# Ensembl/WiggleTools

Measured on AMD Instinct MI355X. Metric: genomic bp/s (whole node) for 'mean' over N BigWig tracks, higher is better.
Workload: dtype f64

## Files before the change

wiggletools_amd/csrc/wt_engine.hip:

```cpp
#include <hip/hip_runtime.h>

#include <cstdio>
#include <thread>
#include <atomic>
#include <cstring>
#include <map>
#include <mutex>
#include <string>
#include <vector>

#include "wt_host.h"
#include "wt_trackset.h"
#include "wt_core.h"
#include "wt_plan.h"
#include "wt_kernels.h"
#include "wt_devscope.h"
#include "wt_pool.h"

#ifndef WT_INDEX_UNROLL
#define WT_INDEX_UNROLL 2
#endif
#define WT_INDEX_CHUNK (256 * 4 * WT_INDEX_UNROLL)
__global__ void __launch_bounds__(256) wt_index_kernel(const WtParams P, long long total, long long span) {
    const long long dev_total = P.seg_off[(long long) P.n_chrom * P.n_tracks];
    if (total > dev_total) total = dev_total;
    const long long begin0 = (long long) blockIdx.x * span;
    long long end0 = begin0 + span;
    if (end0 > total) end0 = total;
    if (begin0 >= end0) return;
    WtIndexCursor cur;
    wt_index_cursor_set(P, cur, wt_index_find_segment(P, begin0));
    struct __attribute__((packed, aligned(4))) V4 { int32_t x[4]; };
    V4 f[WT_INDEX_UNROLL], nf[WT_INDEX_UNROLL];
    int32_t pf[WT_INDEX_UNROLL], npf[WT_INDEX_UNROLL];
    const long long n_full = (end0 - begin0) / WT_INDEX_CHUNK;
    auto fetch = [&](long long base, V4 (&v)[WT_INDEX_UNROLL], int32_t (&p)[WT_INDEX_UNROLL]) {
#pragma unroll
        for (int u = 0; u < WT_INDEX_UNROLL; u++) {
            const long long g = base + 4ll * (threadIdx.x + 256 * u);
            v[u] = *(const V4 *) (P.finish + g);
            p[u] = P.finish[g > 0 ? g - 1 : 0];
        }
    };
    if (n_full > 0) {
        const long long last_full = begin0 + (n_full - 1) * WT_INDEX_CHUNK;
        fetch(begin0, f, pf);
        for (long long begin = begin0; begin <= last_full; begin += WT_INDEX_CHUNK) {
            const long long nb = begin + WT_INDEX_CHUNK;
            fetch(nb <= last_full ? nb : last_full, nf, npf);
#pragma unroll
            for (int u = 0; u < WT_INDEX_UNROLL; u++) {
                const long long g = begin + 4ll * (threadIdx.x + 256 * u);
                int32_t prev = pf[u];
#pragma unroll
                for (int q = 0; q < 4; q++) {
                    wt_index_apply(P, cur, g + q, f[u].x[q], prev);
                    prev = f[u].x[q];
                }
            }
#pragma unroll
            for (int u = 0; u < WT_INDEX_UNROLL; u++) { f[u] = nf[u]; pf[u] = npf[u]; }
        }
    }
    const long long begin = begin0 + n_full * WT_INDEX_CHUNK;
    if (begin < end0) {
#pragma unroll
        for (int u = 0; u < WT_INDEX_UNROLL; u++) {
            const long long g = begin + 4ll * (threadIdx.x + 256 * u);
            int32_t prev = (g < end0 && g > 0) ? P.finish[g - 1] : 0;
#pragma unroll
            for (int q = 0; q < 4; q++) {
                if (g + q < end0) {
                    const int32_t fq = P.finish[g + q];
                    wt_index_apply(P, cur, g + q, fq, prev);
                    prev = fq;
                }
            }
        }
    }
}

#define WT_ISEARCH_ROWS 64
#define WT_ISEARCH_TRACKS 16

__device__ __forceinline__ int wt_index_row_chrom(const WtParams &P, long long row) {
    int lo = 0;
    for (int hi = P.n_chrom; hi - lo > 1;) {
        const int mid = (lo + hi) >> 1;
        if (P.c_first_win[mid] + mid <= row) lo = mid; else hi = mid;
    }
    return lo;
}

struct WtIndexRow { int ch; long long b, s0, n; };
__device__ __forceinline__ WtIndexRow wt_index_row(const WtParams &P, long long row, int i) {
    WtIndexRow r;
    r.ch = P.n_chrom == 1 ? 0 : wt_index_row_chrom(P, row);
    const long long m = row - (P.c_first_win[r.ch] + r.ch);
    const long long seg = (long long) r.ch * P.n_tracks + i;
    r.s0 = P.seg_off[seg];
    r.n = P.seg_off[seg + 1] - r.s0;
    r.b = (long long) P.cbase[r.ch] + (m << P.logW);
    return r;
}

__global__ void __launch_bounds__(256) wt_index_coarse_kernel(const WtParams P, long long n_strips, uint32_t *coarse) {
    const long long t = (long long) blockIdx.x * 256 + threadIdx.x;
    const int N = P.n_tracks;
    if (t >= n_strips * N) return;
    const long long strip = t / N;
    const int i = (int) (t - strip * N);
    const WtIndexRow r = wt_index_row(P, strip * WT_ISEARCH_ROWS, i);
    const int32_t *fin = P.finish + r.s0;
    long long g = r.n >> 1;
    float density = 0.0f;
    if (r.n > 1) {
        const long long f0 = fin[0], f1 = fin[r.n - 1];
        if (f1 > f0) {
            density = (float) (r.n - 1) / (float) (f1 - f0);
            const float guess = fminf(fmaxf((float) (r.b - f0) * density, 0.0f), (float) (r.n - 1));
            g = (long long) guess;
            if (g > r.n - 1) g = r.n - 1;
        }
    }
    coarse[t] = (uint32_t) wt_interp_lower_bound(WtFinArray{fin}, 0, r.n, g, r.b, density);
}

__global__ void __launch_bounds__(WT_ISEARCH_ROWS * WT_ISEARCH_TRACKS) wt_index_search_kernel(const WtParams P, long long n_rows, long long n_strips,
                                                                                              const uint32_t *coarse) {
    __shared__ uint32_t out[WT_ISEARCH_ROWS][WT_ISEARCH_TRACKS + 1];
    const int tid = threadIdx.x, lane = tid & 63;
    const int wave = __builtin_amdgcn_readfirstlane(tid >> 6);
    const int N = P.n_tracks;
    const long long strip = blockIdx.x;
    const long long r0 = strip * WT_ISEARCH_ROWS;
    const int i = (int) blockIdx.y * WT_ISEARCH_TRACKS + wave;
    if (i < N) {
        long long row = r0 + lane;
        if (row > n_rows - 1) row = n_rows - 1;
        const WtIndexRow r = wt_index_row(P, row, i);
        const int32_t *fin = P.finish + r.s0;
        const bool have_next = strip + 1 < n_strips;
        const long long cA = (long long) coarse[strip * N + i];
        const long long cB = have_next ? (long long) coarse[(strip + 1) * N + i] : 0;
        bool real_a = true, real_b = have_next;
        if (P.n_chrom != 1) {
            const int ch_first = __shfl(r.ch, 0);
            const int ch_next = have_next ? wt_index_row_chrom(P, r0 + WT_ISEARCH_ROWS) : -1;
            real_a = r.ch == ch_first; real_b = r.ch == ch_next;
        }
        const long long A = real_a ? cA : 0;
        const long long B = real_b ? cB : r.n;
        long long g = (real_a && real_b) ? A + (((B - A) * lane) >> 6) : (A + B) >> 1;
        if (g > B - 1) g = B - 1;
        const float density = (real_a && real_b) ? (float) (B - A) / (float) ((long long) WT_ISEARCH_ROWS << P.logW) : 0.0f;
        out[lane][wave] = (uint32_t) wt_interp_lower_bound(WtFinArray{fin}, A, B, g, r.b, density);
    }
    __syncthreads();
    const int orow = tid / WT_ISEARCH_TRACKS, ocol = tid % WT_ISEARCH_TRACKS;
    const long long row = r0 + orow;
    const int track = (int) blockIdx.y * WT_ISEARCH_TRACKS + ocol;
    if (row < n_rows && track < N) P.widx[(size_t) row * N + track] = out[orow][ocol];
}

__global__ void __launch_bounds__(256) wt_index_compare_kernel(const uint32_t *a, const uint32_t *b, long long n, unsigned long long *diff) {
    const long long t = (long long) blockIdx.x * 256 + threadIdx.x;
    if (t < n && a[t] != b[t]) atomicAdd(diff, 1ull);
}

__global__ void __launch_bounds__(256) wt_extents_kernel(const int64_t *seg_off, const int32_t *start,
                                                          const int32_t *finish, long long n_seg,
                                                          int32_t *first_start, int32_t *last_finish) {
    const long long s = (long long) blockIdx.x * blockDim.x + threadIdx.x;
    if (s >= n_seg) return;
    const long long lo = seg_off[s], hi = seg_off[s + 1];
    first_start[s] = hi > lo ? start[lo] : 0;
    last_finish[s] = hi > lo ? finish[hi - 1] : 0;
}

__global__ void __launch_bounds__(256) wt_win_chrom_kernel(const int64_t *c_first_win, int n_chrom, long long n_windows, int32_t *win_chrom) {
    const long long k = (long long) blockIdx.x * 256 + threadIdx.x;
    if (k >= n_windows) return;
    int lo = 0;
    for (int hi = n_chrom; hi - lo > 1;) {
        const int mid = (lo + hi) >> 1;
        if (c_first_win[mid] <= k) lo = mid; else hi = mid;
    }
    win_chrom[k] = lo;
}

__global__ void __launch_bounds__(256) wt_clear_kernel(unsigned long long *counters, int n_counters, int64_t *chrom_run_off, int n_cro,
                                                        unsigned long long *status, long long n_status) {
    const long long t = (long long) blockIdx.x * 256 + threadIdx.x, stride = (long long) gridDim.x * 256;
    for (long long q = t; q < n_status; q += stride) status[q] = 0ull;
    for (long long q = t; q < n_counters; q += stride) counters[q] = 0ull;
    for (long long q = t; q < n_cro; q += stride) chrom_run_off[q] = 0;
}

__global__ void __launch_bounds__(256) wt_validate_kernel(const int32_t *start, const int32_t *finish, const int64_t *seg_off,
                                                           long long n_seg, long long total, unsigned long long *out) {
    const long long g = (long long) blockIdx.x * blockDim.x + threadIdx.x;
    if (g >= total) return;
    bool bad = finish[g] <= start[g];
    if (!bad && g > 0 && start[g] < finish[g - 1]) {
        long long lo = 0, hi = n_seg;
        while (hi - lo > 1) {
            const long long mid = (lo + hi) >> 1;
            if (seg_off[mid] <= g) lo = mid; else hi = mid;
        }
        bad = seg_off[lo] != g;
    }
    if (bad) {
        atomicAdd(&out[0], 1ull);
        atomicMin(&out[1], (unsigned long long) g);
    }
}

static thread_local std::string g_last_error;

int wt_fail(int code, const std::string &msg) {
    g_last_error = msg;
    return code;
}

template <class T>
static hipError_t wt_grow(T **p, int64_t *cap, int64_t need, bool *quiet) {
    if (*cap >= need && *p) return hipSuccess;
    int64_t c = *cap * 2;
    if (c < need) c = need;
    if (c < 1) c = 1;
    if (*p) {
        if (!*quiet) {
            const hipError_t eq = wt_pool_quiesce();
            if (eq != hipSuccess) return eq;
            *quiet = true;
        }
        (void) wt_dev_free(*p);
    }
    *p = nullptr; *cap = 0;
    const hipError_t e = wt_dev_alloc(p, sizeof(T) * (size_t) c);
    if (e == hipSuccess) *cap = c;
    return e;
}

static void wt_free_windows(WtWindows &w) {
    (void) wt_dev_free(w.d_tabs);
    (void) wt_dev_free(w.d_widx); (void) wt_dev_free(w.d_cidx); (void) wt_dev_free(w.d_status); (void) wt_dev_free(w.d_bad_list); (void) wt_dev_free(w.d_bad_goff);
    if (w.h_tab) wt_host_free(w.h_tab);
    if (w.ev_tab) (void) hipEventDestroy(w.ev_tab);
    w = WtWindows();
}

extern "C" {

const char *wtamd_last_error(void) { return g_last_error.c_str(); }
const char *wtamd_version(void) { return "wiggletools_amd 0.1 (gfx950)"; }

int wtamd_device_count(void) {
    int n = 0;
    if (hipGetDeviceCount(&n) != hipSuccess) return 0;
    return n;
}

__global__ void wt_warm_kernel(int *p) { if (p && threadIdx.x == 4096) *p = 0; }

static std::mutex g_warm_mu;
static std::thread *g_warm_thread = nullptr;
static bool g_warm_started = false;

extern "C++" void wt_warmup_join() {
    std::thread *t = nullptr;
    { std::lock_guard<std::mutex> lk(g_warm_mu); t = g_warm_thread; g_warm_thread = nullptr; }
    if (t) { t->join(); delete t; }
}

static std::atomic<int> g_device_chosen{-1};

void wtamd_warmup_async(void) {
    std::lock_guard<std::mutex> lk(g_warm_mu);
    if (g_warm_started || getenv("WTAMD_NO_WARMUP")) return;
    int n = 0, cur = -1;
    if (hipGetDeviceCount(&n) != hipSuccess || n <= 0) { (void) hipGetLastError(); return; }
    int ordinal = g_device_chosen.load();
    if (ordinal < 0 && hipGetDevice(&cur) == hipSuccess && (n == 1 || cur > 0)) ordinal = cur;
    if (ordinal < 0 || ordinal >= n) return;
    g_warm_started = true;
    g_warm_thread = new std::thread([ordinal] {
        if (hipSetDevice(ordinal) != hipSuccess) { (void) hipGetLastError(); return; }
        hipStream_t st[3] = {nullptr, nullptr, nullptr};
        for (auto &s : st)
            if (hipStreamCreateWithFlags(&s, hipStreamNonBlocking) != hipSuccess) s = nullptr;
        for (auto &s : st)
            if (s) hipLaunchKernelGGL(wt_warm_kernel, dim3(1), dim3(64), 0, s, (int *) nullptr);
        for (auto &s : st)
            if (s) { (void) hipStreamSynchronize(s); (void) hipStreamDestroy(s); }
        (void) hipGetLastError();
    });
    atexit(wt_warmup_join);
}

int wtamd_set_device(int ordinal) {
    wt_warmup_join();
    WT_HIP(hipSetDevice(ordinal));
    g_device_chosen.store(ordinal);
    return WTAMD_OK;
}

int wtamd_current_device(void) {
    int d = 0;
    if (hipGetDevice(&d) != hipSuccess) { (void) hipGetLastError(); return -1; }
    return d;
}

extern "C++" int wt_trackset_common(const wtamd_tracks *t, wtamd_trackset *ts) {
    if (!t || t->n_chrom < 0 || t->n_tracks <= 0 || !t->seg_off || !t->defaults)
        return wt_fail(WTAMD_ERR_ARG, "wtamd_trackset_create: bad tracks descriptor");
    if (wtamd_device_count() <= 0) return wt_fail(WTAMD_ERR_NODEVICE, "no HIP device visible");
    ts->n_chrom = t->n_chrom;
    ts->n_tracks = t->n_tracks;
    ts->value_f64 = t->value_is_f64 != 0;
    const int64_t n_seg = (int64_t) t->n_chrom * t->n_tracks;
    ts->seg_off.assign(t->seg_off, t->seg_off + n_seg + 1);
    for (int64_t s = 0; s < n_seg; s++)
        if (ts->seg_off[s + 1] < ts->seg_off[s]) return wt_fail(WTAMD_ERR_ARG, "seg_off not monotone");
    ts->n_intervals = ts->seg_off[n_seg] - ts->seg_off[0];
    if (ts->seg_off[0] != 0) return wt_fail(WTAMD_ERR_ARG, "seg_off[0] must be 0");
    ts->defaults.assign(t->defaults, t->defaults + t->n_tracks);
    if (t->range_lo && t->range_hi) {
        ts->range_lo.assign(t->range_lo, t->range_lo + t->n_chrom);
        ts->range_hi.assign(t->range_hi, t->range_hi + t->n_chrom);
    }
    ts->scratch_f32 = !ts->value_f64 && wt_defaults_fit_f32(ts->defaults.data(), ts->n_tracks);
    WT_HIP(hipGetDevice(&ts->device));
    hipDeviceProp_t prop;
    WT_HIP(hipGetDeviceProperties(&prop, ts->device));
    ts->num_cu = prop.multiProcessorCount;
    WT_HIP(wt_dev_alloc(&ts->d_seg_off, sizeof(int64_t) * (n_seg + 1)));
    WT_HIP(hipMemcpy(ts->d_seg_off, ts->seg_off.data(), sizeof(int64_t) * (n_seg + 1), hipMemcpyHostToDevice));
    WT_HIP(wt_dev_alloc(&ts->d_defaults, sizeof(double) * t->n_tracks));
    WT_HIP(hipMemcpy(ts->d_defaults, ts->defaults.data(), sizeof(double) * t->n_tracks, hipMemcpyHostToDevice));
    WT_HIP(wt_dev_alloc(&ts->d_counters, sizeof(unsigned long long) * WT_CTR_N));
    WT_HIP(wt_host_alloc((void **) &ts->h_counters, sizeof(unsigned long long) * WT_CTR_N));
    WT_HIP(wt_host_alloc((void **) &ts->h_debug, sizeof(unsigned long long) * 16));
    memset(ts->h_debug, 0, sizeof(unsigned long long) * 16);
    WT_HIP(wt_dev_alloc(&ts->d_chrom_run_off, sizeof(int64_t) * (t->n_chrom + 1)));
    WT_HIP(hipEventCreate(&ts->ev_i0));
    WT_HIP(hipEventCreate(&ts->ev_i1));
    WT_HIP(hipEventCreate(&ts->ev_r0));
    WT_HIP(hipEventCreate(&ts->ev_r1));
    return WTAMD_OK;
}

extern "C++" int wt_check_extents(wtamd_trackset *ts) {
    for (size_t q = 0; q < ts->last_finish.size(); q++)
        if (ts->seg_off[q + 1] > ts->seg_off[q] && ts->last_finish[q] > WTAMD_MAX_COORD) {
            const int64_t bad = ts->last_finish[q];
            return wt_fail(WTAMD_ERR_ARG, "run finish " + std::to_string(bad) + " above the supported maximum " +
                           std::to_string((long long) WTAMD_MAX_COORD) + " (2^31 - 65537)");
        }
    return WTAMD_OK;
}

static int wt_refresh_extents_device(wtamd_trackset *ts, hipStream_t s) {
    const int64_t n_seg = (int64_t) ts->n_chrom * ts->n_tracks;
    ts->first_start.assign(n_seg, 0);
    ts->last_finish.assign(n_seg, 0);
    if (n_seg > 0 && ts->n_intervals > 0) {
        const size_t bytes = sizeof(int32_t) * 2 * (size_t) n_seg;
        if (!ts->d_extents) WT_HIP(wt_dev_alloc(&ts->d_extents, bytes));
        if (!ts->h_extents) WT_HIP(wt_host_alloc((void **) &ts->h_extents, bytes));
        hipLaunchKernelGGL(wt_extents_kernel, dim3((unsigned) ((n_seg + 255) / 256)), dim3(256), 0, s,
                           ts->d_seg_off, ts->d_start, ts->d_finish, (long long) n_seg, ts->d_extents, ts->d_extents + n_seg);
        WT_HIP(hipGetLastError());
        WT_HIP(hipMemcpyAsync(ts->h_extents, ts->d_extents, bytes, hipMemcpyDeviceToHost, s));
        WT_HIP(hipStreamSynchronize(s));
        ts->first_start.assign(ts->h_extents, ts->h_extents + n_seg);
        ts->last_finish.assign(ts->h_extents + n_seg, ts->h_extents + 2 * n_seg);
    }
    return WTAMD_OK;
}

static int wt_create_host_impl(const wtamd_tracks *t, wtamd_trackset *ts) {
    int rc = wt_trackset_common(t, ts);
    if (rc != WTAMD_OK) return rc;
    ts->owns = true;
    const int64_t n = ts->n_intervals;
    const size_t vsz = ts->value_f64 ? 8 : 4;
    const int64_t n_alloc = n > 0 ? n : 1;
    WT_HIP(hipMalloc(&ts->d_start, sizeof(int32_t) * n_alloc));
    WT_HIP(hipMalloc(&ts->d_finish, sizeof(int32_t) * n_alloc));
    WT_HIP(hipMalloc(&ts->d_value, vsz * n_alloc));
    if (n > 0) {
        if (!t->start || !t->finish || !t->value) return wt_fail(WTAMD_ERR_ARG, "NULL arrays");
        WT_HIP(hipMemcpy(ts->d_start, t->start, sizeof(int32_t) * n, hipMemcpyHostToDevice));
        WT_HIP(hipMemcpy(ts->d_finish, t->finish, sizeof(int32_t) * n, hipMemcpyHostToDevice));
        WT_HIP(hipMemcpy(ts->d_value, t->value, vsz * n, hipMemcpyHostToDevice));
    }
    const int64_t n_seg = (int64_t) ts->n_chrom * ts->n_tracks;
    ts->first_start.assign(n_seg, 0);
    ts->last_finish.assign(n_seg, 0);
    for (int64_t s = 0; s < n_seg; s++)
        if (ts->seg_off[s + 1] > ts->seg_off[s]) {
            ts->first_start[s] = t->start[ts->seg_off[s]];
            ts->last_finish[s] = t->finish[ts->seg_off[s + 1] - 1];
        }
    return wt_check_extents(ts);
}

int wtamd_trackset_create_host(const wtamd_tracks *t, wtamd_trackset **out) {
    if (!out) return wt_fail(WTAMD_ERR_ARG, "out == NULL");
    wtamd_trackset *ts = new wtamd_trackset();
    const int rc = wt_create_host_impl(t, ts);
    if (rc != WTAMD_OK) { wtamd_trackset_destroy(ts); return rc; }
    *out = ts;
    return WTAMD_OK;
}

static int wt_create_device_impl(const wtamd_tracks *t, wtamd_trackset *ts) {
    int rc = wt_trackset_common(t, ts);
    if (rc != WTAMD_OK) return rc;
    ts->owns = false;
    ts->d_start = const_cast<int32_t *>(t->start);
    ts->d_finish = const_cast<int32_t *>(t->finish);
    ts->d_value = const_cast<void *>(t->value);
    rc = wt_refresh_extents_device(ts, nullptr);
    if (rc != WTAMD_OK) return rc;
    return wt_check_extents(ts);
}

int wtamd_trackset_create_device(const wtamd_tracks *t, wtamd_trackset **out) {
    if (!out) return wt_fail(WTAMD_ERR_ARG, "out == NULL");
    wtamd_trackset *ts = new wtamd_trackset();
    const int rc = wt_create_device_impl(t, ts);
    if (rc != WTAMD_OK) { wtamd_trackset_destroy(ts); return rc; }
    *out = ts;
    return WTAMD_OK;
}

void wtamd_trackset_destroy(wtamd_trackset *ts) {
    if (!ts) return;
    (void) wt_pool_quiesce();
    if (ts->owns) { (void) hipFree(ts->d_start); (void) hipFree(ts->d_finish); (void) hipFree(ts->d_value); }
    (void) wt_dev_free(ts->d_seg_off); (void) wt_dev_free(ts->d_defaults); (void) wt_dev_free(ts->d_counters); (void) wt_dev_free(ts->d_chrom_run_off);
    (void) wt_dev_free(ts->d_extents);
    (void) hipFree(ts->d_gscratch); (void) hipFree(ts->d_mwu_table);
    for (double *q : ts->mwu_retired) (void) hipFree(q);
    if (ts->h_counters) wt_host_free(ts->h_counters);
    if (ts->h_debug) wt_host_free(ts->h_debug);
    if (ts->h_extents) wt_host_free(ts->h_extents);
    for (auto &kv : ts->windows) wt_free_windows(kv.second);
    if (ts->ev_i0) (void) hipEventDestroy(ts->ev_i0);
    if (ts->ev_i1) (void) hipEventDestroy(ts->ev_i1);
    if (ts->ev_r0) (void) hipEventDestroy(ts->ev_r0);
    if (ts->ev_r1) (void) hipEventDestroy(ts->ev_r1);
    delete ts;
}

static int64_t wt_span(const wtamd_trackset *ts) {
    int64_t span = 0;
    for (int c = 0; c < ts->n_chrom; c++) {
        int64_t lo = INT64_MAX, hi = INT64_MIN;
        for (int i = 0; i < ts->n_tracks; i++) {
            const int64_t s = (int64_t) c * ts->n_tracks + i;
            if (ts->seg_off[s + 1] > ts->seg_off[s]) {
                lo = std::min<int64_t>(lo, ts->first_start[s]);
                hi = std::max<int64_t>(hi, ts->last_finish[s]);
            }
        }
        if (lo <= hi) span += hi - lo;
    }
    return span;
}

int64_t wtamd_trackset_max_runs(const wtamd_trackset *ts) {
    if (!ts) return 0;
    return std::min<int64_t>(2 * ts->n_intervals, wt_span(ts));
}

static int wt_get_windows(wtamd_trackset *ts, int W, WtWindows **out, hipStream_t s = nullptr) {
    WtWindows &w = ts->windows[W];
    *out = &w;
    if (w.tab_valid) return WTAMD_OK;
    wt_make_windows(ts->n_chrom, ts->n_tracks, ts->seg_off.data(), ts->first_start.data(), ts->last_finish.data(), W, w.tab,
                    ts->range_lo.empty() ? nullptr : ts->range_lo.data(),
                    ts->range_hi.empty() ? nullptr : ts->range_hi.data(), false);
    w.indexed = false;
    const int64_t nc = ts->n_chrom > 0 ? ts->n_chrom : 1;
    const int64_t nwin = w.tab.n_windows > 0 ? w.tab.n_windows : 1;
    const int64_t nwidx = (w.tab.n_rows > 0 ? w.tab.n_rows : 1) * (int64_t) ts->n_tracks;
    auto up8 = [](int64_t x) { return (x + 7) & ~(int64_t) 7; };
    bool quiet = false;
    if (w.cap_chrom < nc || w.cap_win < nwin || !w.d_tabs) {
        const int64_t cc = w.cap_chrom < nc ? std::max<int64_t>(nc, 2 * w.cap_chrom) : w.cap_chrom;
        const int64_t cw = w.cap_win < nwin ? std::max<int64_t>(nwin, 2 * w.cap_win) : w.cap_win;
        const int64_t o_cnwin = up8(4 * cc), o_chi = o_cnwin + up8(4 * cc), o_cfirst = o_chi + up8(4 * cc), o_win = o_cfirst + 8 * (cc + 1);
        const int64_t total = o_win + up8(4 * cw);
        if (w.d_tabs || w.d_status) { WT_HIP(wt_pool_quiesce()); quiet = true; }
        (void) wt_dev_free(w.d_tabs);
        w.d_tabs = nullptr; w.cap_tabs = 0;
        w.d_cbase = w.d_cnwin = w.d_chi = w.d_win_chrom = nullptr; w.d_cfirst = nullptr;
        if (w.cap_win < cw) { (void) wt_dev_free(w.d_status); w.d_status = nullptr; }
        w.cap_chrom = 0; w.cap_win = 0;
        WT_HIP(wt_dev_alloc(&w.d_tabs, (size_t) total));
        if (!w.d_status) WT_HIP(wt_dev_alloc(&w.d_status, sizeof(unsigned long long) * (size_t) cw));
        w.cap_tabs = total;
        w.d_cbase = (int32_t *) w.d_tabs; w.d_cnwin = (int32_t *) (w.d_tabs + o_cnwin); w.d_chi = (int32_t *) (w.d_tabs + o_chi);
        w.d_cfirst = (int64_t *) (w.d_tabs + o_cfirst); w.d_win_chrom = (int32_t *) (w.d_tabs + o_win);
        w.cap_chrom = cc; w.cap_win = cw;
    }
    WT_HIP(wt_grow(&w.d_widx, &w.cap_widx, nwidx, &quiet));
    WT_HIP(wt_grow(&w.d_cidx, &w.cap_cidx, ((w.tab.n_rows > 0 ? w.tab.n_rows : 1) + WT_ISEARCH_ROWS - 1) / WT_ISEARCH_ROWS * (int64_t) ts->n_tracks, &quiet));
    if (ts->n_chrom > 0) {
        if (ts->pipe_mode && ts->n_chrom != 1) return wt_fail(WTAMD_ERR_INTERNAL, "pipeline slots hold one chromosome");
        if (!w.ev_tab) WT_HIP(hipEventCreateWithFlags(&w.ev_tab, hipEventDisableTiming));
        if (w.tab_in_flight) { WT_HIP(hipEventSynchronize(w.ev_tab)); w.tab_in_flight = false; }
        const int64_t head = (char *) w.d_win_chrom - w.d_tabs;
        if (w.h_tab_bytes < head) {
            if (w.h_tab) wt_host_free(w.h_tab);
            w.h_tab = nullptr; w.h_tab_bytes = 0;
            WT_HIP(wt_host_alloc((void **) &w.h_tab, (size_t) head));
            w.h_tab_bytes = head;
        }
        const int64_t o_cfirst = (char *) w.d_cfirst - w.d_tabs;
        const int64_t used = o_cfirst + (int64_t) sizeof(int64_t) * (ts->n_chrom + 1);
        memset(w.h_tab, 0, (size_t) used);
        memcpy(w.h_tab + ((char *) w.d_cbase - w.d_tabs), w.tab.cbase.data(), sizeof(int32_t) * ts->n_chrom);
        memcpy(w.h_tab + ((char *) w.d_cnwin - w.d_tabs), w.tab.c_nwin.data(), sizeof(int32_t) * ts->n_chrom);
        memcpy(w.h_tab + ((char *) w.d_chi - w.d_tabs), w.tab.c_hi.data(), sizeof(int32_t) * ts->n_chrom);
        memcpy(w.h_tab + o_cfirst, w.tab.c_first_win.data(), sizeof(int64_t) * (ts->n_chrom + 1));
        WT_HIP(hipMemcpyAsync(w.d_tabs, w.h_tab, (size_t) used, hipMemcpyHostToDevice, s));
        WT_HIP(hipEventRecord(w.ev_tab, s));
        w.tab_in_flight = true;
        if (w.tab.n_windows > 0) {
            if (ts->n_chrom == 1) {
                WT_HIP(hipMemsetAsync(w.d_win_chrom, 0, sizeof(int32_t) * (size_t) w.tab.n_windows, s));
            } else {
                hipLaunchKernelGGL(wt_win_chrom_kernel, dim3((unsigned) ((w.tab.n_windows + 255) / 256)), dim3(256), 0, s,
                                   (const int64_t *) w.d_cfirst, ts->n_chrom, (long long) w.tab.n_windows, w.d_win_chrom);
                WT_HIP(hipGetLastError());
            }
        }
    }
    w.tab_valid = true;
    return WTAMD_OK;
}

static void wt_fill_params(const wtamd_trackset *ts, const WtWindows *w, const WtPlan &plan, WtParams &P) {
    memset(&P, 0, sizeof(P));
    P.start = ts->d_start; P.finish = ts->d_finish; P.value = ts->d_value;
    P.seg_off = ts->d_seg_off; P.defaults = ts->d_defaults;
    P.n_chrom = ts->n_chrom; P.n_tracks = ts->n_tracks; P.n_total = ts->n_intervals;
    P.cbase = w->d_cbase; P.c_nwin = w->d_cnwin; P.c_hi = w->d_chi; P.c_first_win = w->d_cfirst;
    P.n_windows = w->tab.n_windows; P.win_chrom = w->d_win_chrom; P.widx = w->d_widx;
    P.status = w->d_status; P.counters = ts->d_counters; P.debug = ts->h_debug;
    wt_plan_to_params(plan, P);
}

static int wt_build_index(wtamd_trackset *ts, WtWindows *w, const WtPlan &plan, hipStream_t s) {
    WtParams P;
    wt_fill_params(ts, w, plan, P);
    WT_HIP(hipEventRecord(ts->ev_i0, s));
    static const int mode = [] {
        const char *e = getenv("WTAMD_INDEX"), *c = getenv("WTAMD_INDEX_CHECK");
        if (c && atoi(c) > 0) return 2;
        return (e && !strcmp(e, "scan")) ? 1 : 0;
    }();
    const size_t n_widx = (size_t) w->tab.n_rows * ts->n_tracks;
    auto scan = [&](uint32_t *dst) -> int {
        WtParams Q = P;
        Q.widx = dst;
        WT_HIP(hipMemsetAsync(dst, 0, sizeof(uint32_t) * n_widx, s));
        if (ts->n_intervals > 0) {
            const long long total = ts->n_intervals;
            long long blocks = (total + WT_INDEX_CHUNK - 1) / WT_INDEX_CHUNK;
            const long long cap = (long long) ts->num_cu * 8;
            if (blocks > cap) blocks = cap;
            long long span = (total + blocks - 1) / blocks;
            span = (span + WT_INDEX_CHUNK - 1) / WT_INDEX_CHUNK * WT_INDEX_CHUNK;
            blocks = (total + span - 1) / span;
            hipLaunchKernelGGL(wt_index_kernel, dim3((unsigned) blocks), dim3(256), 0, s, Q, total, span);
            WT_HIP(hipGetLastError());
        }
        return WTAMD_OK;
    };
    auto search = [&](uint32_t *dst) -> int {
        WtParams Q = P;
        Q.widx = dst;
        const long long n_rows = w->tab.n_rows;
        if (n_rows > 0 && ts->n_tracks > 0) {
            const long long n_strips = (n_rows + WT_ISEARCH_ROWS - 1) / WT_ISEARCH_ROWS;
            if (w->cap_cidx < n_strips * ts->n_tracks) return wt_fail(WTAMD_ERR_INTERNAL, "coarse window index not allocated");
            hipLaunchKernelGGL(wt_index_coarse_kernel, dim3((unsigned) ((n_strips * ts->n_tracks + 255) / 256)), dim3(256), 0, s, Q, n_strips, w->d_cidx);
            WT_HIP(hipGetLastError());
            const dim3 grid((unsigned) n_strips, (unsigned) ((ts->n_tracks + WT_ISEARCH_TRACKS - 1) / WT_ISEARCH_TRACKS));
            hipLaunchKernelGGL(wt_index_search_kernel, grid, dim3(WT_ISEARCH_ROWS * WT_ISEARCH_TRACKS), 0, s, Q, n_rows, n_strips, (const uint32_t *) w->d_cidx);
            WT_HIP(hipGetLastError());
        }
        return WTAMD_OK;
    };
    if (mode == 1) {
        if (int rc = scan(w->d_widx)) return rc;
    } else {
        if (int rc = search(w->d_widx)) return rc;
    }
    if (mode == 2 && n_widx > 0) {
        uint32_t *other = nullptr;
        unsigned long long *d_diff = nullptr, h_diff = 0;
        WT_HIP(hipMalloc(&other, sizeof(uint32_t) * n_widx));
        WT_HIP(hipMalloc(&d_diff, sizeof(unsigned long long)));
        WT_HIP(hipMemsetAsync(d_diff, 0, sizeof(unsigned long long), s));
        if (int rc = scan(other)) return rc;
        hipLaunchKernelGGL(wt_index_compare_kernel, dim3((unsigned) ((n_widx + 255) / 256)), dim3(256), 0, s, w->d_widx, other, (long long) n_widx, d_diff);
        WT_HIP(hipMemcpyAsync(&h_diff, d_diff, sizeof(h_diff), hipMemcpyDeviceToHost, s));
        WT_HIP(hipStreamSynchronize(s));
        (void) hipFree(other); (void) hipFree(d_diff);
        if (h_diff) {
            fprintf(stderr, "wiggletools_amd: WTAMD_INDEX_CHECK: the searched window index differs from the scanned one in %llu of %zu entries\n", h_diff, n_widx);
            return wt_fail(WTAMD_ERR_INTERNAL, "window index check failed");
        }
    }
    WT_HIP(hipEventRecord(ts->ev_i1, s));
    ts->have_index_time = true;
    w->indexed = true;
    return WTAMD_OK;
}

static inline int wt_delta_class(int op) { return op == WT_OP_TTEST ? 1 : ((op == WT_OP_MAX || op == WT_OP_MIN) ? 2 : 0); }
static bool wt_wants_delta(const wtamd_trackset *ts, int op) {
    return !ts->delta_failed_[wt_delta_class(op)] && wt_delta_eligible(op, ts->value_f64, ts->n_tracks, ts->defaults.data());
}

static double wt_events_per_bp(const wtamd_trackset *ts) {
    const int64_t span = wt_span(ts);
    return span > 0 ? 1.25 * (double) ts->n_intervals / (double) span : 0.0;
}

static bool wt_mwu_few_ties(wtamd_trackset *ts, hipStream_t stream) {
    if (ts->mwu_few_ties >= 0) return ts->mwu_few_ties != 0;
    ts->mwu_few_ties = 0;
    if (hipStreamSynchronize(stream) != hipSuccess) { (void) hipGetLastError(); return false; }
    const int64_t n = ts->n_intervals;
    if (n < 1024 || ts->value_f64 || !ts->d_value) return false;
    const int64_t S = std::min<int64_t>(4096, n), stride = n / S;
    std::vector<uint32_t> v((size_t) S);
    if (hipMemcpy2D(v.data(), 4, ts->d_value, (size_t) stride * 4, 4, (size_t) S, hipMemcpyDeviceToHost) != hipSuccess) { (void) hipGetLastError(); return false; }
    std::sort(v.begin(), v.end());
    const int64_t distinct = (int64_t) (std::unique(v.begin(), v.end()) - v.begin());
    ts->mwu_few_ties = distinct * 100 >= S * 97 ? 1 : 0;
    return ts->mwu_few_ties != 0;
}

static bool wt_pick_plan(wtamd_trackset *ts, int op, int n_set0, WtPlan &plan, std::string &err, hipStream_t stream = nullptr) {
    static const int mwalk = getenv("WTAMD_MWALK") ? (atoi(getenv("WTAMD_MWALK")) != 0 ? 1 : 0) : -1;
    const bool walk = !getenv("WTAMD_NO_WALK");
    const bool mwu_walk = op == WT_OP_MWU && mwalk != 0 && !ts->value_f64 && walk && (mwalk == 1 || wt_mwu_few_ties(ts, stream));
    const double events_per_bp = (op == WT_OP_MEDIAN || op == WT_OP_MWU) ? wt_events_per_bp(ts) : 0.0;
    return wt_pick_general_plan(ts->n_tracks, op, ts->value_f64, ts->scratch_f32, n_set0, walk, mwu_walk, events_per_bp, plan, err);
}

static void wt_trackset_forget(wtamd_trackset *ts, bool delta_failed) {
    for (int q = 0; q < 3; q++) { ts->delta_verified_[q] = false; ts->delta_failed_[q] = delta_failed; ts->delta_n_bad_[q] = 0; }
    for (auto &kv : ts->windows) kv.second.indexed = false;
}

extern "C++" int wt_trackset_rebind(wtamd_trackset *ts, int64_t n, const int64_t *seg_off, int32_t range_lo, int32_t range_hi, bool value_f64,
                                    int32_t *d_start, int32_t *d_finish, void *d_value, bool delta_failed) {
    ts->n_intervals = n;
    ts->seg_off.assign(seg_off, seg_off + (int64_t) ts->n_chrom * ts->n_tracks + 1);
    ts->range_lo[0] = range_lo;
    ts->range_hi[0] = range_hi;
    ts->value_f64 = value_f64;
    ts->scratch_f32 = !ts->value_f64 && wt_defaults_fit_f32(ts->defaults.data(), ts->n_tracks);
    ts->d_start = d_start; ts->d_finish = d_finish; ts->d_value = d_value;
    wt_trackset_forget(ts, delta_failed);
    for (auto &kv : ts->windows) kv.second.tab_valid = false;
    return wt_check_extents(ts);
}

int wtamd_trackset_index(wtamd_trackset *ts, int op, void *stream) {
    if (!ts) return wt_fail(WTAMD_ERR_ARG, "ts == NULL");
    wt_trackset_forget(ts, false);
    ts->mwu_few_ties = -1;
    if (!ts->owns && !ts->pipe_mode) {
        int rce = wt_refresh_extents_device(ts, (hipStream_t) stream);
        if (rce != WTAMD_OK) return rce;
        rce = wt_check_extents(ts);
        if (rce != WTAMD_OK) return rce;
        for (auto &kv : ts->windows) kv.second.tab_valid = false;
    }
    WtPlan plan;
    std::string err;
    if (wt_wants_delta(ts, op)) wt_make_delta_plan_for(plan, ts->n_tracks, op);
    else if (!wt_pick_plan(ts, op, ts->n_tracks / 2, plan, err, (hipStream_t) stream)) return wt_fail(WTAMD_ERR_ARG, err);
    WtWindows *w = nullptr;
    int rc = wt_get_windows(ts, plan.W, &w, (hipStream_t) stream);
    if (rc != WTAMD_OK) return rc;
    return wt_build_index(ts, w, plan, (hipStream_t) stream);
}

extern "C++" int wt_check_desc(const wtamd_trackset *ts, const wtamd_reduce_desc *d) {
    if (!ts || !d) return wt_fail(WTAMD_ERR_ARG, "NULL argument");
    if (d->op < 0 || d->op >= WTAMD_OP_COUNT_) return wt_fail(WTAMD_ERR_ARG, "unknown op");
    if (d->op == WTAMD_OP_TTEST) {
        if (d->n_set0 < 3 || ts->n_tracks - d->n_set0 < 3)
            return wt_fail(WTAMD_ERR_ARG, "The t-test function only works for two sets with enough elements to compute variance");
    } else if (d->op == WTAMD_OP_MWU) {
        if (d->n_set0 < 1 || ts->n_tracks - d->n_set0 < 1)
            return wt_fail(WTAMD_ERR_ARG, "The Mann-Whitney U function only works for two non-empty sets");
    }
    return WTAMD_OK;
}

static int wt_reduce_plan(wtamd_trackset *ts, const WtPlan &plan, int op, uint32_t flags, int n_set0, wtamd_runs *runs,
                          double *d_tile, uint8_t *d_inplay, int64_t *n_runs, hipStream_t s);

extern "C++" int wt_launch_patch(wtamd_trackset *ts, int delta_W, int op, uint32_t flags, int n_set0, wtamd_runs *runs, long long n_bad,
                                 hipStream_t s) {
    WtPlan plan;
    std::string err;
    if (!wt_make_plan(ts->n_tracks, op, ts->scratch_f32, plan, err)) return wt_fail(WTAMD_ERR_INTERNAL, err);
    if (!wt_patch_compatible(plan, delta_W, ts->scratch_f32, ts->value_f64))
        return wt_fail(WTAMD_ERR_INTERNAL, "no general plan compatible with the difference-array windows (general W " + std::to_string(plan.W) + ", difference-array W " +
                       std::to_string(delta_W) + ", slab " + std::to_string((long long) plan.scratch_slab) + ", float staging " + std::to_string((int) ts->scratch_f32) + ", f64 values " +
                       std::to_string((int) ts->value_f64) + ")");
    WtWindows *dw = nullptr, *w = nullptr;
    int rc = wt_get_windows(ts, delta_W, &dw, s);
    if (rc != WTAMD_OK) return rc;
    rc = wt_get_windows(ts, plan.W, &w, s);
    if (rc != WTAMD_OK) return rc;
    WtLaunch L;
    WtParams &P = L.P;
    wt_fill_params(ts, w, plan, P);
    P.op = op; P.flags = flags; P.n_set0 = op == WT_OP_TTEST ? n_set0 : 0;
    P.capacity = runs->capacity;
    P.o_start = runs->start; P.o_finish = runs->finish; P.o_value = runs->value;
    P.chrom_run_off = runs->chrom_run_off ? runs->chrom_run_off : ts->d_chrom_run_off;
    L.T = plan.T; L.lds = plan.lds_bytes; L.stream = s; L.num_cu = ts->num_cu;
    WtPatchArgs Q;
    Q.bad_list = dw->d_bad_list; Q.bad_goff = dw->d_bad_goff;
    Q.n_bad = ts->d_counters + WT_CTR_DELTA_BAD;
    Q.d_win_chrom = dw->d_win_chrom; Q.d_c_first_win = dw->d_cfirst;
    Q.ratio = delta_W / plan.W;
    if (!wt_patch_launch(L, Q, op, plan.ppt, plan.n_chunks > 1, n_bad, !w->indexed))
        return wt_fail(WTAMD_ERR_INTERNAL, "no general plan compatible with the difference-array windows");
    if (L.err != hipSuccess) return wt_fail(WTAMD_ERR_HIP, std::string("patch kernel launch: ") + hipGetErrorString(L.err));
    WT_HIP(hipEventRecord(ts->ev_r1, s));
    ts->stats.patched_windows = (int32_t) n_bad;
    return WTAMD_OK;
}

static int wt_reduce_impl(wtamd_trackset *ts, int op, uint32_t flags, int n_set0, wtamd_runs *runs,
                          double *d_tile, uint8_t *d_inplay, int64_t *n_runs, hipStream_t s) {
    if (!runs || !runs->start || !runs->finish || !runs->value)
        return wt_fail(WTAMD_ERR_ARG, "wtamd_reduce: output arrays missing");
    WtPlan plan;
    std::string err;
    if (!d_tile && wt_wants_delta(ts, op)) {
        wt_make_delta_plan_for(plan, ts->n_tracks, op);
        const int dc = wt_delta_class(op);
        int64_t n_probe = 0;
        const bool probe = !ts->delta_verified_[dc];
        const int rc = wt_reduce_plan(ts, plan, op, flags, n_set0, runs, d_tile, d_inplay,
                                      (probe && !n_runs) ? &n_probe : n_runs, s);
        if (!probe) {
            if (ts->delta_n_bad_[dc] > 0 && (rc == WTAMD_OK || rc == WTAMD_ERR_CAPACITY)) {
                const int rp = wt_launch_patch(ts, plan.W, op, flags, n_set0, runs, ts->delta_n_bad_[dc], s);
                if (rp != WTAMD_OK) return rp;
                if (n_runs) WT_HIP(hipStreamSynchronize(s));
            }
            return rc;
        }
        if (rc != WTAMD_OK && rc != WTAMD_ERR_CAPACITY) return rc;
        const long long n_bad = (long long) ts->h_counters[WT_CTR_DELTA_BAD];
        if (n_bad == 0) { ts->delta_verified_[dc] = true; ts->delta_n_bad_[dc] = 0; return rc; }
        if (wt_few_enough_to_patch(n_bad, ts->stats.n_windows) && !getenv("WTAMD_NO_PATCH")) {
            const int rp = wt_launch_patch(ts, plan.W, op, flags, n_set0, runs, n_bad, s);
            if (rp == WTAMD_OK) {
                WT_HIP(hipStreamSynchronize(s));
                ts->delta_verified_[dc] = true;
                ts->delta_n_bad_[dc] = n_bad;
                return rc;
            }
            if (rp != WTAMD_ERR_INTERNAL) return rp;
        }
        ts->delta_failed_[dc] = true;
    }
    if (!wt_pick_plan(ts, op, n_set0, plan, err, s)) return wt_fail(WTAMD_ERR_ARG, err);
    return wt_reduce_plan(ts, plan, op, flags, n_set0, runs, d_tile, d_inplay, n_runs, s);
}

extern "C++" int wt_reduce_enqueue(wtamd_trackset *ts, const wtamd_reduce_desc &desc, wtamd_runs *runs, double *d_tile, uint8_t *d_inplay,
                                   hipStream_t s, bool *used_delta, int *delta_W) {
    WtPlan plan;
    std::string err;
    *used_delta = !d_tile && wt_wants_delta(ts, desc.op);
    if (*used_delta) {
        wt_make_delta_plan_for(plan, ts->n_tracks, desc.op);
        *delta_W = plan.W;
    } else if (!wt_pick_plan(ts, desc.op, desc.n_set0, plan, err, s)) {
        return wt_fail(WTAMD_ERR_ARG, err);
    }
    return wt_reduce_plan(ts, plan, desc.op, desc.flags, desc.n_set0, runs, d_tile, d_inplay, nullptr, s);
}

static int wt_reduce_plan(wtamd_trackset *ts, const WtPlan &plan, int op, uint32_t flags, int n_set0, wtamd_runs *runs,
                          double *d_tile, uint8_t *d_inplay, int64_t *n_runs, hipStream_t s) {
    if (plan.T > (plan.delta ? ((wt_op_is_var_family(op) || op == WT_OP_TTEST) ? wt_delta_sq_block : wt_delta_block) : wt_reduce_max_block)) return wt_fail(WTAMD_ERR_ARG, "workgroup size above the kernel's launch bound");
    WtWindows *w = nullptr;
    int rc = wt_get_windows(ts, plan.W, &w, s);
    if (rc != WTAMD_OK) return rc;
    if (!w->indexed) {
        rc = wt_build_index(ts, w, plan, s);
        if (rc != WTAMD_OK) return rc;
    }
    WtLaunch L;
    wt_fill_params(ts, w, plan, L.P);
    L.P.op = op; L.P.flags = flags; L.P.n_set0 = n_set0;
    L.P.capacity = runs->capacity;
    L.P.o_start = runs->start; L.P.o_finish = runs->finish; L.P.o_value = runs->value;
    L.P.chrom_run_off = runs->chrom_run_off ? runs->chrom_run_off : ts->d_chrom_run_off;
    L.P.o_tile = d_tile; L.P.o_inplay = d_inplay;
    L.T = plan.T; L.lds = plan.lds_bytes; L.stream = s; L.num_cu = ts->num_cu;
    L.gscratch = &ts->d_gscratch; L.gscratch_bytes = &ts->gscratch_bytes;
    if (op == WT_OP_MWU && !getenv("WTAMD_MWU_DEVICE_ERF")) {
        const int n1 = n_set0, n2 = ts->n_tracks - n_set0;
        if (ts->mwu_n1 != n1 || ts->mwu_n2 != n2) {
            std::vector<double> t;
            const bool have = wt_mwu_make_table(n1, n2, t);
            if (ts->d_mwu_table) { ts->mwu_retired.push_back(ts->d_mwu_table); ts->d_mwu_table = nullptr; }
            if (have) {
                WT_HIP(hipMalloc((void **) &ts->d_mwu_table, sizeof(double) * t.size()));
                WT_HIP(hipMemcpyAsync(ts->d_mwu_table, t.data(), sizeof(double) * t.size(), hipMemcpyHostToDevice, s));
                WT_HIP(hipStreamSynchronize(s));
            }
            ts->mwu_n1 = n1; ts->mwu_n2 = n2; ts->mwu_kmax = have ? (int) t.size() - 1 : 0;
        }
        L.P.mwu_table = ts->d_mwu_table;
        L.P.mwu_kmax = ts->mwu_kmax;
    }
    if (plan.delta) {
        const int64_t nwin = w->tab.n_windows > 0 ? w->tab.n_windows : 1;
        if (w->cap_bad < nwin) {
            int64_t c1 = w->cap_bad, c2 = w->cap_bad;
// ... 254 lines not shown
```

wiggletools_amd/csrc/wt_isearch.h:

```cpp
#ifndef WT_ISEARCH_H_
#define WT_ISEARCH_H_

#include <math.h>
#include <stdint.h>

#ifndef WT_DEV
#if defined(__HIPCC__) && !defined(WT_EMU)
#define WT_DEV __device__ __forceinline__
#else
#define WT_DEV inline
#endif
#endif

struct WtFinArray {
    const int32_t *p;
    WT_DEV long long operator()(long long x) const { return (long long) p[x]; }
};

template <class Fin>
WT_DEV long long wt_gallop_lower_bound(Fin fin, long long lo, long long hi, long long g, long long b) {
    if (lo >= hi) return lo;
    if (fin(g) >= b) {
        hi = g;
        for (long long d = 1;; d <<= 1) {
            const long long q = hi - d;
            if (q < lo) break;
            if (fin(q) < b) { lo = q + 1; break; }
            hi = q;
        }
    } else {
        lo = g + 1;
        for (long long d = 1;; d <<= 1) {
            const long long q = lo + d - 1;
            if (q >= hi) break;
            if (fin(q) >= b) { hi = q; break; }
            lo = q + 1;
        }
    }
    while (lo < hi) {
        const long long mid = (lo + hi) >> 1;
        if (fin(mid) < b) lo = mid + 1; else hi = mid;
    }
    return lo;
}

#define WT_ISEARCH_STEPS 2
template <class Fin>
WT_DEV long long wt_interp_lower_bound(Fin fin, long long lo, long long hi, long long g, long long b, float density) {
    if (lo >= hi) return lo;
    if (density > 0.0f) {
        for (int step = 0; step < WT_ISEARCH_STEPS; step++) {
            const long long f = fin(g);
            if (f >= b) hi = g; else lo = g + 1;
            if (lo >= hi) return lo;
            const float span = (float) (hi - lo);
            const float move = fminf(fmaxf((float) (b - f) * density, -span), span);
            g += (long long) move;
            if (g < lo) g = lo;
            if (g > hi - 1) g = hi - 1;
        }
    }
    return wt_gallop_lower_bound(fin, lo, hi, g, b);
}

WT_DEV long long wt_lane_lower_bound(const int32_t *fin, long long lo, long long hi, long long g, long long b) {
    return wt_gallop_lower_bound(WtFinArray{fin}, lo, hi, g, b);
}

#endif
```

wiggletools_amd/csrc/wt_trackset.h:

```cpp
#ifndef WT_TRACKSET_H_
#define WT_TRACKSET_H_

#include <map>
#include <vector>

#include "wt_host.h"
#include "wt_plan.h"

struct WtWindows {
    WtPlan plan_geom;
    WtWindowTables tab;
    int32_t *d_cbase = nullptr, *d_cnwin = nullptr, *d_chi = nullptr, *d_win_chrom = nullptr;
    int64_t *d_cfirst = nullptr;
    uint32_t *d_widx = nullptr;
    uint32_t *d_cidx = nullptr;
    unsigned long long *d_status = nullptr;
    int32_t *d_bad_list = nullptr;
    long long *d_bad_goff = nullptr;
    bool indexed = false;
    int64_t cap_chrom = 0, cap_win = 0, cap_widx = 0, cap_bad = 0, cap_cidx = 0;
    bool tab_valid = false;
    char *h_tab = nullptr;
    int64_t h_tab_bytes = 0;
    hipEvent_t ev_tab = nullptr;
    bool tab_in_flight = false;
    char *d_tabs = nullptr;
    int64_t cap_tabs = 0;
};

struct wtamd_trackset {
    int n_chrom = 0, n_tracks = 0;
    bool value_f64 = false;
    bool owns = false;
    int64_t n_intervals = 0;
    std::vector<int64_t> seg_off;
    std::vector<double> defaults;
    std::vector<int32_t> first_start, last_finish;
    std::vector<int32_t> range_lo, range_hi;
    int32_t *d_start = nullptr, *d_finish = nullptr;
    void *d_value = nullptr;
    int64_t *d_seg_off = nullptr;
    double *d_defaults = nullptr;
    unsigned long long *d_counters = nullptr;
    unsigned long long *h_counters = nullptr;
    unsigned long long *h_debug = nullptr;
    int64_t *d_chrom_run_off = nullptr;
    int32_t *d_extents = nullptr, *h_extents = nullptr;
    char *d_gscratch = nullptr;
    size_t gscratch_bytes = 0;
    double *d_mwu_table = nullptr;
    int mwu_n1 = -1, mwu_n2 = -1, mwu_kmax = 0;
    int mwu_few_ties = -1;
    std::vector<double *> mwu_retired;
    std::map<int, WtWindows> windows;
    hipEvent_t ev_i0 = nullptr, ev_i1 = nullptr, ev_r0 = nullptr, ev_r1 = nullptr;
    bool have_index_time = false, have_reduce_time = false;
    wtamd_stats stats{};
    int device = 0;
    int num_cu = 256;
    bool scratch_f32 = false;
    bool delta_failed_[3] = {false, false, false};
    bool delta_verified_[3] = {false, false, false};
    long long delta_n_bad_[3] = {0, 0, 0};
    bool pipe_mode = false;
};

void wt_warmup_join();
int wt_trackset_common(const wtamd_tracks *t, wtamd_trackset *ts);
int wt_check_extents(wtamd_trackset *ts);
int wt_check_desc(const wtamd_trackset *ts, const wtamd_reduce_desc *d);

int wt_trackset_rebind(wtamd_trackset *ts, int64_t n, const int64_t *seg_off, int32_t range_lo, int32_t range_hi, bool value_f64,
                       int32_t *d_start, int32_t *d_finish, void *d_value, bool delta_failed);

int wt_reduce_enqueue(wtamd_trackset *ts, const wtamd_reduce_desc &desc, wtamd_runs *runs, double *d_tile, uint8_t *d_inplay,
                      hipStream_t s, bool *used_delta, int *delta_W);

int wt_launch_patch(wtamd_trackset *ts, int delta_W, int op, uint32_t flags, int n_set0, wtamd_runs *runs, long long n_bad,
                    hipStream_t s);

#endif
```

Baseline: 49.38 billion.

## Write extents to pinned host memory with seq-flag polling; build one-chrom tables in one kernel

The extents kernel now writes first/last coordinates straight into pinned host memory. Its last block publishes a sequence number with a system-scope release, and the host spin-polls that word instead of doing a memcpy and a stream synchronize. The single-chromosome window-table path replaces the host table upload and memset with one kernel that fills the tables on device. A wide block-scan interpolation lower-bound helper is added but not called here. The changes target per-call host latency and add spin-wait CPU use plus a dependence on correct cross-block atomics.

```diff
diff --git a/wiggletools_amd/csrc/wt_engine.hip b/wiggletools_amd/csrc/wt_engine.hip
--- a/wiggletools_amd/csrc/wt_engine.hip
+++ b/wiggletools_amd/csrc/wt_engine.hip
@@ -170,12 +170,22 @@
 
 __global__ void __launch_bounds__(256) wt_extents_kernel(const int64_t *seg_off, const int32_t *start,
                                                           const int32_t *finish, long long n_seg,
-                                                          int32_t *first_start, int32_t *last_finish) {
+                                                          int32_t *first_start, int32_t *last_finish,
+                                                          unsigned *count, unsigned long long *seq_word, unsigned long long seq) {
     const long long s = (long long) blockIdx.x * blockDim.x + threadIdx.x;
-    if (s >= n_seg) return;
-    const long long lo = seg_off[s], hi = seg_off[s + 1];
-    first_start[s] = hi > lo ? start[lo] : 0;
-    last_finish[s] = hi > lo ? finish[hi - 1] : 0;
+    if (s < n_seg) {
+        const long long lo = seg_off[s], hi = seg_off[s + 1];
+        first_start[s] = hi > lo ? start[lo] : 0;
+        last_finish[s] = hi > lo ? finish[hi - 1] : 0;
+    }
+    __threadfence_system();
+    __syncthreads();
+    if (threadIdx.x != 0) return;
+    if (gridDim.x > 1) {
+        if (__hip_atomic_fetch_add(count, 1u, __ATOMIC_ACQ_REL, __HIP_MEMORY_SCOPE_AGENT) != gridDim.x - 1) return;
+        __hip_atomic_store(count, 0u, __ATOMIC_RELAXED, __HIP_MEMORY_SCOPE_AGENT);
+    }
+    __hip_atomic_store(seq_word, seq, __ATOMIC_RELEASE, __HIP_MEMORY_SCOPE_SYSTEM);
 }
 
 __global__ void __launch_bounds__(256) wt_win_chrom_kernel(const int64_t *c_first_win, int n_chrom, long long n_windows, int32_t *win_chrom) {
@@ -187,6 +197,13 @@
         if (c_first_win[mid] <= k) lo = mid; else hi = mid;
     }
     win_chrom[k] = lo;
+}
+
+__global__ void __launch_bounds__(256) wt_one_chrom_tables_kernel(int32_t *cbase, int32_t *c_nwin, int32_t *c_hi, int64_t *c_first_win, int32_t *win_chrom,
+                                                                   int32_t cbase0, int32_t c_nwin0, int32_t c_hi0, long long n_windows) {
+    const long long t = (long long) blockIdx.x * 256 + threadIdx.x, stride = (long long) gridDim.x * 256;
+    for (long long k = t; k < n_windows; k += stride) win_chrom[k] = 0;
+    if (t == 0) { cbase[0] = cbase0; c_nwin[0] = c_nwin0; c_hi[0] = c_hi0; c_first_win[0] = 0; c_first_win[1] = n_windows; }
 }
 
 __global__ void __launch_bounds__(256) wt_clear_kernel(unsigned long long *counters, int n_counters, int64_t *chrom_run_off, int n_cro,
@@ -366,14 +383,36 @@
     ts->first_start.assign(n_seg, 0);
     ts->last_finish.assign(n_seg, 0);
     if (n_seg > 0 && ts->n_intervals > 0) {
-        const size_t bytes = sizeof(int32_t) * 2 * (size_t) n_seg;
-        if (!ts->d_extents) WT_HIP(wt_dev_alloc(&ts->d_extents, bytes));
-        if (!ts->h_extents) WT_HIP(wt_host_alloc((void **) &ts->h_extents, bytes));
-        hipLaunchKernelGGL(wt_extents_kernel, dim3((unsigned) ((n_seg + 255) / 256)), dim3(256), 0, s,
-                           ts->d_seg_off, ts->d_start, ts->d_finish, (long long) n_seg, ts->d_extents, ts->d_extents + n_seg);
+        const size_t o_seq = (sizeof(int32_t) * 2 * (size_t) n_seg + 7) & ~(size_t) 7;
+        const unsigned blocks = (unsigned) ((n_seg + 255) / 256);
+        if (!ts->h_extents) {
+            WT_HIP(wt_host_alloc((void **) &ts->h_extents, o_seq + sizeof(unsigned long long)));
+            *(unsigned long long *) ((char *) ts->h_extents + o_seq) = 0ull;
+            ts->extents_seq = 0;
+        }
+        if (blocks > 1 && !ts->d_extents_count) {
+            WT_HIP(wt_dev_alloc(&ts->d_extents_count, sizeof(unsigned)));
+            WT_HIP(hipMemsetAsync(ts->d_extents_count, 0, sizeof(unsigned), s));
+        }
+        unsigned long long *seq_word = (unsigned long long *) ((char *) ts->h_extents + o_seq);
+        const unsigned long long seq = ++ts->extents_seq;
+        hipLaunchKernelGGL(wt_extents_kernel, dim3(blocks), dim3(256), 0, s,
+                           ts->d_seg_off, ts->d_start, ts->d_finish, (long long) n_seg, ts->h_extents, ts->h_extents + n_seg,
+                           ts->d_extents_count, seq_word, seq);
         WT_HIP(hipGetLastError());
-        WT_HIP(hipMemcpyAsync(ts->h_extents, ts->d_extents, bytes, hipMemcpyDeviceToHost, s));
-        WT_HIP(hipStreamSynchronize(s));
+        unsigned looks = 0;
+        const int rcw = wt_bounded_wait([&]() -> hipError_t {
+            if (__atomic_load_n(seq_word, __ATOMIC_ACQUIRE) == seq) return hipSuccess;
+            if (++looks & 1023u) return hipErrorNotReady;
+            const hipError_t q = hipStreamQuery(s);
+            if (q != hipSuccess) return q;
+            return __atomic_load_n(seq_word, __ATOMIC_ACQUIRE) == seq ? hipSuccess : hipErrorUnknown;
+        }, "extents", "the sequence number of wt_extents_kernel", 0.002, 200, [seq](double limit_s) {
+            char buf[160];
+            snprintf(buf, sizeof buf, "the extents kernel did not report its sequence number %llu within %.0f s", seq, limit_s);
+            return std::string(buf);
+        });
+        if (rcw != WTAMD_OK) return rcw;
         ts->first_start.assign(ts->h_extents, ts->h_extents + n_seg);
         ts->last_finish.assign(ts->h_extents + n_seg, ts->h_extents + 2 * n_seg);
     }
@@ -442,7 +481,7 @@
     (void) wt_pool_quiesce();
     if (ts->owns) { (void) hipFree(ts->d_start); (void) hipFree(ts->d_finish); (void) hipFree(ts->d_value); }
     (void) wt_dev_free(ts->d_seg_off); (void) wt_dev_free(ts->d_defaults); (void) wt_dev_free(ts->d_counters); (void) wt_dev_free(ts->d_chrom_run_off);
-    (void) wt_dev_free(ts->d_extents);
+    (void) wt_dev_free(ts->d_extents_count);
     (void) hipFree(ts->d_gscratch); (void) hipFree(ts->d_mwu_table);
     for (double *q : ts->mwu_retired) (void) hipFree(q);
     if (ts->h_counters) wt_host_free(ts->h_counters);
@@ -510,8 +549,15 @@
     }
     WT_HIP(wt_grow(&w.d_widx, &w.cap_widx, nwidx, &quiet));
     WT_HIP(wt_grow(&w.d_cidx, &w.cap_cidx, ((w.tab.n_rows > 0 ? w.tab.n_rows : 1) + WT_ISEARCH_ROWS - 1) / WT_ISEARCH_ROWS * (int64_t) ts->n_tracks, &quiet));
-    if (ts->n_chrom > 0) {
-        if (ts->pipe_mode && ts->n_chrom != 1) return wt_fail(WTAMD_ERR_INTERNAL, "pipeline slots hold one chromosome");
+    if (ts->pipe_mode && ts->n_chrom != 1) return wt_fail(WTAMD_ERR_INTERNAL, "pipeline slots hold one chromosome");
+    if (ts->n_chrom == 1) {
+        const long long nw = w.tab.n_windows;
+        const unsigned blocks = (unsigned) std::min<long long>(std::max<long long>((nw + 255) / 256, 1), 1024);
+        hipLaunchKernelGGL(wt_one_chrom_tables_kernel, dim3(blocks), dim3(256), 0, s, w.d_cbase, w.d_cnwin, w.d_chi, w.d_cfirst, w.d_win_chrom,
+                           w.tab.cbase[0], w.tab.c_nwin[0], w.tab.c_hi[0], nw);
+        WT_HIP(hipGetLastError());
+    }
+    if (ts->n_chrom > 1) {
         if (!w.ev_tab) WT_HIP(hipEventCreateWithFlags(&w.ev_tab, hipEventDisableTiming));
         if (w.tab_in_flight) { WT_HIP(hipEventSynchronize(w.ev_tab)); w.tab_in_flight = false; }
         const int64_t head = (char *) w.d_win_chrom - w.d_tabs;
@@ -532,13 +578,9 @@
         WT_HIP(hipEventRecord(w.ev_tab, s));
         w.tab_in_flight = true;
         if (w.tab.n_windows > 0) {
-            if (ts->n_chrom == 1) {
-                WT_HIP(hipMemsetAsync(w.d_win_chrom, 0, sizeof(int32_t) * (size_t) w.tab.n_windows, s));
-            } else {
-                hipLaunchKernelGGL(wt_win_chrom_kernel, dim3((unsigned) ((w.tab.n_windows + 255) / 256)), dim3(256), 0, s,
-                                   (const int64_t *) w.d_cfirst, ts->n_chrom, (long long) w.tab.n_windows, w.d_win_chrom);
-                WT_HIP(hipGetLastError());
-            }
+            hipLaunchKernelGGL(wt_win_chrom_kernel, dim3((unsigned) ((w.tab.n_windows + 255) / 256)), dim3(256), 0, s,
+                               (const int64_t *) w.d_cfirst, ts->n_chrom, (long long) w.tab.n_windows, w.d_win_chrom);
+            WT_HIP(hipGetLastError());
         }
     }
     w.tab_valid = true;
diff --git a/wiggletools_amd/csrc/wt_isearch.h b/wiggletools_amd/csrc/wt_isearch.h
--- a/wiggletools_amd/csrc/wt_isearch.h
+++ b/wiggletools_amd/csrc/wt_isearch.h
@@ -15,6 +15,14 @@
 struct WtFinArray {
     const int32_t *p;
     WT_DEV long long operator()(long long x) const { return (long long) p[x]; }
+    WT_DEV int misalign() const { return (int) (((uintptr_t) p >> 2) & 15u); }
+    WT_DEV void quad(long long x, long long (&v)[4]) const {
+        struct __attribute__((aligned(16))) Q4 { int32_t e[4]; };
+        const Q4 q = *(const Q4 *) (p + x);
+        v[0] = q.e[0]; v[1] = q.e[1]; v[2] = q.e[2]; v[3] = q.e[3];
+    }
+    WT_DEV long long edge(long long x) const { return (long long) p[x]; }
+    WT_DEV void begin_wide() const {}
 };
 
 template <class Fin>
@@ -63,6 +71,55 @@
     return wt_gallop_lower_bound(fin, lo, hi, g, b);
 }
 
+#define WT_ISEARCH_BLOCK 16
+template <class Fin>
+WT_DEV long long wt_interp_wide_lower_bound(Fin fin, long long lo, long long hi, long long g, long long b, float density, long long r_lo,
+                                            long long r_hi) {
+    if (lo >= hi) return lo;
+    if (density > 0.0f) {
+        for (int step = 0; step < WT_ISEARCH_STEPS; step++) {
+            const long long f = fin(g);
+            if (f >= b) hi = g; else lo = g + 1;
+            if (lo >= hi) return lo;
+            const float span = (float) (hi - lo);
+            const float move = fminf(fmaxf((float) (b - f) * density, -span), span);
+            g += (long long) move;
+            if (g < lo) g = lo;
+            if (g > hi - 1) g = hi - 1;
+        }
+    }
+    fin.begin_wide();
+    const long long mis = fin.misalign();
+    const long long xb = ((g + mis) & ~(long long) (WT_ISEARCH_BLOCK - 1)) - mis;
+    const long long c0 = xb > lo ? xb : lo, c1 = xb + WT_ISEARCH_BLOCK < hi ? xb + WT_ISEARCH_BLOCK : hi;
+    int below = 0;
+    for (int q = 0; q < WT_ISEARCH_BLOCK / 4; q++) {
+        const long long xs = xb + 4 * q;
+        if (xs >= r_lo && xs + 4 <= r_hi) {
+            long long v[4];
+            fin.quad(xs, v);
+            for (int e = 0; e < 4; e++) below += (int) ((xs + e < lo) | ((xs + e < hi) & (v[e] < b)));
+        } else {
+            for (int e = 0; e < 4; e++) {
+                const long long x = xs + e;
+                if (x < lo) below++;
+                else if (x < hi) below += (int) (fin.edge(x) < b);
+            }
+        }
+    }
+    const long long x = xb + below;
+    if (x <= c0) {
+        if (c0 == lo) return lo;
+        hi = c0; g = c0 - 1;
+    } else if (x >= c1) {
+        if (c1 == hi) return hi;
+        lo = c1; g = c1;
+    } else {
+        return x;
+    }
+    return wt_gallop_lower_bound(fin, lo, hi, g, b);
+}
+
 WT_DEV long long wt_lane_lower_bound(const int32_t *fin, long long lo, long long hi, long long g, long long b) {
     return wt_gallop_lower_bound(WtFinArray{fin}, lo, hi, g, b);
 }
diff --git a/wiggletools_amd/csrc/wt_trackset.h b/wiggletools_amd/csrc/wt_trackset.h
--- a/wiggletools_amd/csrc/wt_trackset.h
+++ b/wiggletools_amd/csrc/wt_trackset.h
@@ -45,7 +45,9 @@
     unsigned long long *h_counters = nullptr;
     unsigned long long *h_debug = nullptr;
     int64_t *d_chrom_run_off = nullptr;
-    int32_t *d_extents = nullptr, *h_extents = nullptr;
+    int32_t *h_extents = nullptr;
+    unsigned long long extents_seq = 0;
+    unsigned *d_extents_count = nullptr;
     char *d_gscratch = nullptr;
     size_t gscratch_bytes = 0;
     double *d_mwu_table = nullptr;
```

Result: no change. 49.65 billion, median of 6 (+0.5%).
